# sk4161/EgoScaler

Hardware: AMD Instinct MI355X
Metric: clips/sec/GPU (8-frame 224^2, 16-token text) fwd+bwd (higher is better)
Workload: dtype bf16

## Files before the change

egoscaler_amd/csrc/api.hip:

```cpp
#include "common.h"

thread_local int egomi_launch_err_ = 0;
thread_local int egomi_last_hip_error_ = 0;

extern "C" int egomi_version(void) { return 100; }

extern "C" const char* egomi_last_launch_error(void) { return hipGetErrorString((hipError_t)egomi_last_hip_error_); }

extern "C" const char* egomi_strerror(int code) {
    switch (code) {
        case EGOMI_OK: return "ok";
        case EGOMI_E_BADARG: return "bad argument (null pointer, unknown dtype/enum)";
        case EGOMI_E_SHAPE: return "shape/stride/workspace check failed";
        case EGOMI_E_LAUNCH: return "HIP launch failed";
        case EGOMI_E_UNSUPPORTED: return "size or mode not supported by this kernel";
        default: return "unknown egomi error";
    }
}

thread_local hipEvent_t egomi_time_start_ = nullptr, egomi_time_stop_ = nullptr;

extern "C" int egomi_event_create(void** event) {
    if (!event) return EGOMI_E_BADARG;
    hipEvent_t e;
// ... 5 lines not shown
extern "C" int egomi_event_destroy(void* event) {
    if (!event) return EGOMI_E_BADARG;
    return hipEventDestroy((hipEvent_t)event) == hipSuccess ? EGOMI_OK : EGOMI_E_LAUNCH;
}
extern "C" int egomi_event_elapsed_ms(void* start, void* stop, float* ms) {
    if (!start || !stop || !ms) return EGOMI_E_BADARG;
    hipError_t rc = hipEventSynchronize((hipEvent_t)stop);
    if (rc == hipSuccess) rc = hipEventElapsedTime(ms, (hipEvent_t)start, (hipEvent_t)stop);
    if (rc != hipSuccess) {
        egomi_last_hip_error_ = (int)rc;
        (void)hipGetLastError();
        return EGOMI_E_LAUNCH;
    }
    return EGOMI_OK;
}
thread_local int egomi_route_[5] = {0, 1, 0, 0, 0};

extern "C" int egomi_gemm_last_route(int* out4) {
    if (!out4) return EGOMI_E_BADARG;
    for (int i = 0; i < 4; ++i) out4[i] = egomi_route_[i + 1];
    return egomi_route_[0];
}

extern "C" int egomi_gemm_time_next(void* start, void* stop) {
    if ((start == nullptr) != (stop == nullptr)) return EGOMI_E_BADARG;
    egomi_time_start_ = (hipEvent_t)start; egomi_time_stop_ = (hipEvent_t)stop;
    return EGOMI_OK;
}
```

egoscaler_amd/csrc/common.h:

```cpp
#pragma once
#include <hip/hip_runtime.h>
#include <stdint.h>
#include "../../include/egomi.h"

typedef uint16_t bf16_t;
typedef __attribute__((ext_vector_type(8))) __bf16 bf16x8;
typedef __attribute__((ext_vector_type(4))) __bf16 bf16x4;
typedef __attribute__((ext_vector_type(4))) float f32x4;
typedef __attribute__((ext_vector_type(16))) float f32x16;
typedef __attribute__((ext_vector_type(4))) uint32_t u32x4;
typedef __attribute__((ext_vector_type(2))) uint32_t u32x2;
typedef __attribute__((ext_vector_type(2))) float f32x2;

#define EGOMI_WAVE 64

__device__ __forceinline__ float bf2f(bf16_t u) { return __uint_as_float(((uint32_t)u) << 16); }
__device__ __forceinline__ bf16_t f2bf(float f) {
    __bf16 h = (__bf16)f;
    return *reinterpret_cast<bf16_t*>(&h);
}

__device__ __forceinline__ void swiglu_bwd_elem(float d, float g, float u, float& og, float& ou) {
#pragma clang fp contract(off)
    const float sg = 1.0f / (1.0f + __expf(-g));
// ... 69 lines not shown
    if ((threadIdx.x & 63) == 0) red[w] = v;
    __syncthreads();
    float t = red[0];
    for (int i = 1; i < nw; ++i) t = fmaxf(t, red[i]);
    return t;
}

__device__ __forceinline__ float act_apply(float x, int act) {
    if (act == 1) return 0.5f * x * (1.0f + erff(x * 0.70710678118654752440f));
    if (act == 2) return fmaxf(x, 0.0f);
    return x;
}

extern thread_local int egomi_launch_err_;
extern thread_local int egomi_last_hip_error_;
#define EGOMI_LAUNCH(...)                                              \
    do {                                                               \
        (void)hipGetLastError();                                       \
        hipLaunchKernelGGL(__VA_ARGS__);                               \
        const hipError_t e_ = hipGetLastError();                       \
        if (e_ != hipSuccess) { egomi_launch_err_ = 1; egomi_last_hip_error_ = (int)e_; } \
    } while (0)
extern thread_local int egomi_route_[5];
static inline void egomi_route_set(int form, int splitk, int row0, int slices, int na) {
    egomi_route_[0] = form; egomi_route_[1] = splitk; egomi_route_[2] = row0; egomi_route_[3] = slices; egomi_route_[4] = na;
}
static inline int egomi_launch_status() {
    const int e = egomi_launch_err_;
    egomi_launch_err_ = 0;
    return e ? EGOMI_E_LAUNCH : EGOMI_OK;
}

#define EGOMI_DISPATCH_DTYPE(dtype, ...)                         \
    do {                                                         \
        if ((dtype) == EGOMI_F32) { typedef float T; __VA_ARGS__; }        \
        else if ((dtype) == EGOMI_BF16) { typedef bf16_t T; __VA_ARGS__; } \
        else return EGOMI_E_BADARG;                              \
    } while (0)
```

egoscaler_amd/csrc/gemm.hip:

```cpp
#include "common.h"

#define GT_BM 128
#define GT_BN 128
#define GT_THREADS 256

template <typename T> struct GemmCfg;
template <> struct GemmCfg<bf16_t> { static constexpr int BK = 64, VEC = 8, LDK = 72; };
template <> struct GemmCfg<float> { static constexpr int BK = 16, VEC = 4, LDK = 17; };

struct GemmArgs {
    const void* A; const void* B; void* C; const void* bias; const void* residual;
    int M, N, K;
    long long lda, ldb, ldc, ldr;
    int batch_inner;
    long long sA0, sA1, sB0, sB1, sC0, sC1;
    float alpha; int accumulate; int act;
};


template <typename T, bool TR, int ROWS>
struct Stager {
    static constexpr int BK = GemmCfg<T>::BK, VEC = GemmCfg<T>::VEC, LDK = GemmCfg<T>::LDK;
    static constexpr int NV = ROWS * BK / VEC / GT_THREADS;
    T v[NV][VEC];
// ... 140 lines not shown
    g.alpha = d->alpha; g.accumulate = d->accumulate; g.act = d->act;
    constexpr int VEC = GemmCfg<T>::VEC;
    auto aligned = [&](const void* p, long long ld, long long s0, long long s1) {
        return ((uintptr_t)p % 16 == 0) && (ld % VEC == 0) && (s0 % VEC == 0) && (s1 % VEC == 0);
    };
    const bool aa = aligned(d->A, d->lda, d->sA0, d->sA1), ba = aligned(d->B, d->ldb, d->sB0, d->sB1);
    dim3 grid((d->N + GT_BN - 1) / GT_BN, (d->M + GT_BM - 1) / GT_BM, d->batch > 0 ? d->batch : 1);
    dim3 block(GT_THREADS);
    const bool TA = d->a_layout == 1, TB = d->b_layout == 1;
    if (!TA && !TB) EGOMI_LAUNCH((gemm_generic_kernel<T, TC, false, false>), grid, block, 0, s, g, aa, ba);
    else if (!TA && TB) EGOMI_LAUNCH((gemm_generic_kernel<T, TC, false, true>), grid, block, 0, s, g, aa, ba);
    else if (TA && !TB) EGOMI_LAUNCH((gemm_generic_kernel<T, TC, true, false>), grid, block, 0, s, g, aa, ba);
    else EGOMI_LAUNCH((gemm_generic_kernel<T, TC, true, true>), grid, block, 0, s, g, aa, ba);
    egomi_route_set(1, 1, d->M, 0, 0);
    return egomi_launch_status();
}

int egomi_gemm_fast_try(const egomi_gemm_desc* d, hipStream_t s);
int egomi_gemm_tn_try(const egomi_gemm_desc* d, hipStream_t s);
extern thread_local hipEvent_t egomi_time_start_, egomi_time_stop_;

extern "C" int egomi_gemm(const egomi_gemm_desc* d, egomi_stream_t stream) {
    egomi_route_set(0, 1, d ? d->M : 0, 0, 0);
    if (!d || !d->A || !d->B || !d->C) return EGOMI_E_BADARG;
    if (d->M <= 0 || d->N <= 0 || d->K <= 0) return EGOMI_E_SHAPE;
    if (d->a_layout < 0 || d->a_layout > 1 || d->b_layout < 0 || d->b_layout > 1 || d->act < 0 || d->act > 2) return EGOMI_E_BADARG;
    const long long min_lda = d->a_layout == 0 ? d->K : d->M, min_ldb = d->b_layout == 0 ? d->K : d->N;
    if (d->lda < min_lda || d->ldb < min_ldb || d->ldc < d->N || (d->residual && d->ldr < d->N)) return EGOMI_E_SHAPE;
    if (d->batch > 65535) return EGOMI_E_UNSUPPORTED;
    hipStream_t s = (hipStream_t)stream;
    if (!d->force_generic) {
        const int r = egomi_gemm_fast_try(d, s);
        if (r <= 0) return r;
        const int r2 = egomi_gemm_tn_try(d, s);
        if (r2 <= 0) return r2;
    } else {
        egomi_time_start_ = egomi_time_stop_ = nullptr;
    }
    if (d->epilogue != EGOMI_EPI_NONE) return EGOMI_E_UNSUPPORTED;
    if (d->ab_dtype == EGOMI_F32 && d->c_dtype == EGOMI_F32) return launch_generic<float, float>(d, s);
    if (d->ab_dtype == EGOMI_BF16 && d->c_dtype == EGOMI_BF16) return launch_generic<bf16_t, bf16_t>(d, s);
    if (d->ab_dtype == EGOMI_BF16 && d->c_dtype == EGOMI_F32) return launch_generic<bf16_t, float>(d, s);
    return EGOMI_E_UNSUPPORTED;
}
```

egoscaler_amd/csrc/gemm_fast.hip:

```cpp
#include "common.h"
#include <mutex>
#include <queue>
#include <unordered_map>
#include <vector>

#define FT_BK 64

struct FastArgs {
    const bf16_t* A; const bf16_t* B; void* C; const bf16_t* bias; const void* residual;
    int M, N, K;
    long long lda, ldb, ldc, ldr;
    float alpha; int accumulate; int act;
    int tiles_m, tiles_n;
    int splitk; float* ws;
    int full_tm, full_tiles, tail_s;
    int epi; void* C2; long long ldc2;
    int* tickets;
};

typedef __attribute__((address_space(3))) void lds_void;
typedef __attribute__((address_space(1))) const void gbl_void;

__device__ __forceinline__ void glds16(const bf16_t* g, bf16_t* lds_wave_base) {
    __builtin_amdgcn_global_load_lds((gbl_void*)g, (lds_void*)lds_wave_base, 16, 0, 0);
// ... 388 lines not shown
                for (int i = 0; i < 4; ++i)
                    acc[j][i] = __builtin_amdgcn_mfma_f32_16x16x32_bf16(fb[ks][j], fa[ks][i], acc[j][i], 0, 0, 0);
    }
    asm volatile("s_waitcnt vmcnt(0)" ::: "memory");
    gemm_epilogue<TC, 4>(g, acc, wm, n0 + wn, lane, g.splitk > 1 ? g.ws + (long long)blockIdx.y * g.M * g.N : nullptr, 0);
}

#ifdef GEMM_STAMP
__device__ unsigned long long g_gemm_stamp[16];
extern "C" int egomi_gemm_stamp_read(unsigned long long* out) { return (int)hipMemcpyFromSymbol(out, HIP_SYMBOL(g_gemm_stamp), sizeof(g_gemm_stamp)); }
extern "C" int egomi_gemm_stamp_reset() { unsigned long long z[16] = {0}; return (int)hipMemcpyToSymbol(HIP_SYMBOL(g_gemm_stamp), z, sizeof(z)); }
#define GSTAMP_DECL unsigned long long gs_prev = 0, gs_acc[6] = {0, 0, 0, 0, 0, 0};
#define GSTAMP_NOW(var) { __builtin_amdgcn_sched_barrier(0); asm volatile("s_memtime %0\n\ts_waitcnt lgkmcnt(0)" : "=s"(var) :: "memory"); __builtin_amdgcn_sched_barrier(0); }
#define GSTAMP_START GSTAMP_NOW(gs_prev)
#define GSTAMP(i) { unsigned long long gs_n; GSTAMP_NOW(gs_n) gs_acc[i] += gs_n - gs_prev; gs_prev = gs_n; }
#define GSTAMP_FLUSH if (threadIdx.x == 0) { for (int i = 0; i < 6; ++i) atomicAdd(&g_gemm_stamp[i], gs_acc[i]); atomicAdd(&g_gemm_stamp[8], 1ull); }
#else
#define GSTAMP_DECL
#define GSTAMP_START
#define GSTAMP(i)
#define GSTAMP_FLUSH
#endif
#define P8_HT (128 * 64)
template <typename TC>
__global__ __launch_bounds__(512, 2)
void gemm_nt_bf16_8phase_kernel(FastArgs g) {
    __shared__ __attribute__((aligned(16))) bf16_t smem[2 * 4 * P8_HT];
    const int lane = threadIdx.x & 63;
    const int wave = __builtin_amdgcn_readfirstlane(threadIdx.x >> 6);
    const int wr = wave >> 2, wc = wave & 3;

    GSTAMP_DECL
    GSTAMP_START
    int tm, tn, kz = 0, ksl = 1;
    if ((int)blockIdx.x < g.full_tiles) {
        const int nwg = g.full_tiles;
        int bid = blockIdx.x;
        const int xcd = bid & 7, q = nwg >> 3, r = nwg & 7;
        bid = (xcd < r ? xcd * (q + 1) : r * (q + 1) + (xcd - r) * q) + (bid >> 3);
        const int per_group = 8 * g.tiles_n;
        const int grp = bid / per_group, first_tm = grp * 8;
        const int gsz = (g.full_tm - first_tm) < 8 ? (g.full_tm - first_tm) : 8;
        const int in_g = bid - grp * per_group;
        tm = first_tm + in_g % gsz; tn = in_g / gsz;
    } else {
        const int idx = blockIdx.x - g.full_tiles, rows = g.tiles_m - g.full_tm;
        ksl = g.tail_s;
        kz = idx % ksl;
        const int tile = idx / ksl;
        tm = g.full_tm + tile % rows; tn = tile / rows;
    }
    const int m0 = tm * 256, n0 = tn * 256;

    unsigned offA[2][2], offB[2][2];
#pragma unroll
    for (int h = 0; h < 2; ++h)
#pragma unroll
        for (int i = 0; i < 2; ++i) {
            const int lr = (wave * 2 + i) * 8 + (lane >> 3);
            const int chunk = (lane & 7) ^ ((lr >> 1) & 7);
            int ra = m0 + (lr >> 6) * 128 + h * 64 + (lr & 63); ra = ra < g.M ? ra : g.M - 1;
            int rb = n0 + (lr >> 5) * 64 + h * 32 + (lr & 31);  rb = rb < g.N ? rb : g.N - 1;
            offA[h][i] = (unsigned)(ra * g.lda + chunk * 8);
            offB[h][i] = (unsigned)(rb * g.ldb + chunk * 8);
        }

    f32x4 acc[4][8];
#pragma unroll
    for (int j = 0; j < 4; ++j)
#pragma unroll
        for (int i = 0; i < 8; ++i) acc[j][i] = (f32x4){0.f, 0.f, 0.f, 0.f};

    const int sw = ((lane & 15) >> 1) & 7, c0 = lane >> 4;
    int aBase[2], bBase[2];
#pragma unroll
    for (int ks = 0; ks < 2; ++ks) {
        aBase[ks] = (wr * 64 + (lane & 15)) * 64 + (((c0 + 4 * ks) ^ sw) << 3);
        bBase[ks] = (wc * 32 + (lane & 15)) * 64 + (((c0 + 4 * ks) ^ sw) << 3);
    }

    int nt = g.K / FT_BK, t_begin = 0;
    if (ksl > 1) {
        const int per = (nt + ksl - 1) / ksl;
        t_begin = kz * per;
        nt = t_begin + per < nt ? t_begin + per : nt;
    }
    const int t_last = nt - 1;

    bf16x8 fa[2][4], fb0[2][2], fb1[2][2];

#define P8_RD(off) (*reinterpret_cast<const bf16x8*>(smem + (off)))
#define P8_LDA(b, X) _Pragma("unroll") for (int ks = 0; ks < 2; ++ks) _Pragma("unroll") for (int ii = 0; ii < 4; ++ii) \
        fa[ks][ii] = P8_RD(((b) * 4 + (X)) * P8_HT + aBase[ks] + ii * 16 * 64);
#define P8_LDB(dst, b, X) _Pragma("unroll") for (int ks = 0; ks < 2; ++ks) _Pragma("unroll") for (int jj = 0; jj < 2; ++jj) \
        dst[ks][jj] = P8_RD(((b) * 4 + 2 + (X)) * P8_HT + bBase[ks] + jj * 16 * 64);
#define P8_PF(b, slot, base, off) _Pragma("unroll") for (int i = 0; i < 2; ++i) \
        glds16((base) + (off)[i], smem + ((b) * 4 + (slot)) * P8_HT + (wave * 2 + i) * 8 * 64);
#define P8_MMA(mh, fbv, nh) __builtin_amdgcn_s_setprio(1); \
        _Pragma("unroll") for (int ks = 0; ks < 2; ++ks) _Pragma("unroll") for (int jj = 0; jj < 2; ++jj) _Pragma("unroll") for (int ii = 0; ii < 4; ++ii) \
            acc[(nh) * 2 + jj][(mh) * 4 + ii] = __builtin_amdgcn_mfma_f32_16x16x32_bf16(fbv[ks][jj], fa[ks][ii], acc[(nh) * 2 + jj][(mh) * 4 + ii], 0, 0, 0); \
        __builtin_amdgcn_s_setprio(0);
#define P8_BAR __builtin_amdgcn_sched_barrier(0); __builtin_amdgcn_s_barrier(); __builtin_amdgcn_sched_barrier(0);
#define P8_TILE(b, tt) { \
        const int t1 = (tt) + 1 < t_last ? (tt) + 1 : t_last, t2 = (tt) + 2 < t_last ? (tt) + 2 : t_last; \
        const bf16_t* pA1 = g.A + (long long)t1 * FT_BK; \
        const bf16_t* pA2 = g.A + (long long)t2 * FT_BK; \
        const bf16_t* pB2 = g.B + (long long)t2 * FT_BK; \
         P8_LDB(fb0, b, 0) __builtin_amdgcn_sched_barrier(0); P8_LDA(b, 0) P8_PF((b) ^ 1, 1, pA1, offA[1]) \
        asm volatile("s_waitcnt lgkmcnt(8)" ::: "memory"); P8_BAR P8_MMA(0, fb0, 0) P8_BAR \
         P8_LDB(fb1, b, 1) P8_PF(b, 2, pB2, offB[0]) P8_BAR P8_MMA(0, fb1, 1) P8_BAR \
         P8_LDA(b, 1) P8_PF(b, 0, pA2, offA[0]) P8_BAR P8_MMA(1, fb1, 1) P8_BAR \
         P8_PF(b, 3, pB2, offB[1]) asm volatile("s_waitcnt vmcnt(6)" ::: "memory"); P8_BAR P8_MMA(1, fb0, 0) P8_BAR \
    }

    {
        const int t1 = t_begin + 1 < t_last ? t_begin + 1 : t_last;
        const bf16_t* pA0 = g.A + (long long)t_begin * FT_BK;
        const bf16_t* pB0 = g.B + (long long)t_begin * FT_BK;
        const bf16_t* pA1 = g.A + (long long)t1 * FT_BK;
        const bf16_t* pB1 = g.B + (long long)t1 * FT_BK;
        P8_PF(0, 2, pB0, offB[0]) P8_PF(0, 0, pA0, offA[0]) P8_PF(0, 3, pB0, offB[1]) P8_PF(0, 1, pA0, offA[1])
        P8_PF(1, 2, pB1, offB[0]) P8_PF(1, 0, pA1, offA[0]) P8_PF(1, 3, pB1, offB[1])
        GSTAMP(0)
        asm volatile("s_waitcnt vmcnt(6)" ::: "memory");
        P8_BAR
        GSTAMP(1)
    }
    if (wr == 1) { P8_BAR }
    int t = t_begin;
    for (; t + 1 < nt; t += 2) {
        P8_TILE(0, t)
        P8_TILE(1, t + 1)
    }
    if (t < nt) P8_TILE(0, t)
    if (wr == 0) { P8_BAR }
    GSTAMP(2)
    asm volatile("s_waitcnt vmcnt(0)" ::: "memory");
    __builtin_amdgcn_s_barrier();
    GSTAMP(3)
    const int row0 = g.full_tm * 256;
    const int mb = m0 + wr * 128, nb = n0 + wc * 64;
    if (ksl > 1 && g.tickets) {
        const int tile = (blockIdx.x - g.full_tiles) / ksl;
        char* slab = reinterpret_cast<char*>(g.ws) + (long long)tile * ksl * 262144;
        {
            __amdgpu_buffer_rsrc_t r = __builtin_amdgcn_make_buffer_rsrc(slab + ((long long)kz * 8 + wave) * 32768, 0, 32768, 0x00020000);
#pragma unroll
            for (int j = 0; j < 4; ++j)
#pragma unroll
                for (int i = 0; i < 8; ++i)
                    __builtin_amdgcn_raw_buffer_store_b128(__builtin_bit_cast(u32x4, acc[j][i]), r, ((j * 8 + i) * 64 + lane) * 16, 0, 16);
        }
        int* flag = reinterpret_cast<int*>(smem);
        asm volatile("s_waitcnt vmcnt(0)" ::: "memory");
        __builtin_amdgcn_s_barrier();
        if (threadIdx.x == 0) *flag = __hip_atomic_fetch_add(g.tickets + tile, 1, __ATOMIC_RELAXED, __HIP_MEMORY_SCOPE_AGENT);
        asm volatile("s_waitcnt vmcnt(0) lgkmcnt(0)" ::: "memory");
        __builtin_amdgcn_s_barrier();
        const int tk = *const_cast<volatile int*>(flag);
        if (tk != ksl - 1) return;
        if (threadIdx.x == 0) __hip_atomic_store(g.tickets + tile, 0, __ATOMIC_RELAXED, __HIP_MEMORY_SCOPE_AGENT);
        const bool all = ksl > 2;
        if (all) {
#pragma unroll
            for (int j = 0; j < 4; ++j)
// ... 7 lines not shown
            for (int j = 0; j < 4; ++j)
#pragma unroll
                for (int i = 0; i < 8; ++i)
                    acc[j][i] += __builtin_bit_cast(f32x4, __builtin_amdgcn_raw_buffer_load_b128(r, ((j * 8 + i) * 64 + lane) * 16, 0, 16));
        }
        gemm_epilogue<TC, 8>(g, acc, mb, nb, lane);
        return;
    }
    if (sizeof(TC) == 2 && ksl == 1 && !g.bias && !g.residual && !g.accumulate && g.act == 0 && g.alpha == 1.0f &&
        nb + 64 <= g.N && (g.ldc & 7) == 0 && ((uintptr_t)g.C & 15) == 0) {
        char* wb = reinterpret_cast<char*>(smem) + wave * (64 * 144);
        bf16_t* C = reinterpret_cast<bf16_t*>(g.C);
        if (g.epi == 3) {
            char* ws3 = reinterpret_cast<char*>(smem) + wave * (32 * 272);
            const bf16_t* GU = reinterpret_cast<const bf16_t*>(g.C2);
            const int lr = lane >> 4, ch = lane & 15;
            u32x4 in[8];
#define P8_GU_FETCH(sp_) _Pragma("unroll") for (int it = 0; it < 8; ++it) { \
                    int m_ = mb + (sp_) * 32 + it * 4 + lr; \
                    m_ = m_ < g.M ? m_ : g.M - 1; \
                    in[it] = *reinterpret_cast<const u32x4*>(GU + (long long)m_ * g.ldc2 + 2 * nb + ch * 8); }
            P8_GU_FETCH(0)
#pragma unroll
            for (int sp = 0; sp < 4; ++sp) {
#pragma unroll
                for (int it = 0; it < 8; ++it) *reinterpret_cast<u32x4*>(ws3 + (it * 4 + lr) * 272 + ch * 16) = in[it];
                if (sp < 3) { P8_GU_FETCH(sp + 1) }
#pragma unroll
                for (int i2 = 0; i2 < 2; ++i2)
#pragma unroll
                    for (int j = 0; j < 4; ++j) {
                        const f32x4 v = acc[j][2 * sp + i2];
                        char* pg = ws3 + (i2 * 16 + (lane & 15)) * 272 + ((j >> 1) * 64 + (j & 1) * 16 + lr * 4) * 2;
                        const u32x2 gg = *reinterpret_cast<const u32x2*>(pg), uu = *reinterpret_cast<const u32x2*>(pg + 64);
                        float og[4], ou[4];
#pragma unroll
                        for (int r = 0; r < 4; ++r) {
                            const float gv = __uint_as_float((r & 1) ? (gg[r >> 1] & 0xFFFF0000u) : (gg[r >> 1] << 16));
                            const float uv = __uint_as_float((r & 1) ? (uu[r >> 1] & 0xFFFF0000u) : (uu[r >> 1] << 16));
                            swiglu_bwd_elem(bf2f(f2bf(v[r])), gv, uv, og[r], ou[r]);
                        }
                        u32x2 o;
                        o[0] = (uint32_t)f2bf(og[0]) | ((uint32_t)f2bf(og[1]) << 16);
                        o[1] = (uint32_t)f2bf(og[2]) | ((uint32_t)f2bf(og[3]) << 16);
                        *reinterpret_cast<u32x2*>(pg) = o;
                        o[0] = (uint32_t)f2bf(ou[0]) | ((uint32_t)f2bf(ou[1]) << 16);
                        o[1] = (uint32_t)f2bf(ou[2]) | ((uint32_t)f2bf(ou[3]) << 16);
                        *reinterpret_cast<u32x2*>(pg + 64) = o;
                    }
#pragma unroll
                for (int it = 0; it < 8; ++it) {
                    const int m = mb + sp * 32 + it * 4 + lr;
                    const u32x4 v = *reinterpret_cast<const u32x4*>(ws3 + (it * 4 + lr) * 272 + ch * 16);
                    if (m < g.M) *reinterpret_cast<u32x4*>(C + (long long)m * g.ldc + 2 * nb + ch * 8) = v;
                }
            }
#undef P8_GU_FETCH
            GSTAMP(4)
            GSTAMP(5)
            GSTAMP_FLUSH
            return;
        }
#pragma unroll
        for (int pass = 0; pass < 2; ++pass) {
#pragma unroll
            for (int ii = 0; ii < 4; ++ii)
#pragma unroll
                for (int j = 0; j < 4; ++j) {
                    const f32x4 v = acc[j][4 * pass + ii];
                    u32x2 o;
                    o[0] = (uint32_t)f2bf(v[0]) | ((uint32_t)f2bf(v[1]) << 16);
                    o[1] = (uint32_t)f2bf(v[2]) | ((uint32_t)f2bf(v[3]) << 16);
                    *reinterpret_cast<u32x2*>(wb + (ii * 16 + (lane & 15)) * 144 + (j * 16 + (lane >> 4) * 4) * 2) = o;
                }
#pragma unroll
            for (int it = 0; it < 8; ++it) {
                const int r = it * 8 + (lane >> 3), ch = lane & 7;
                const u32x4 v = *reinterpret_cast<const u32x4*>(wb + r * 144 + ch * 16);
                const int m = mb + pass * 64 + r;
                if (m < g.M) *reinterpret_cast<u32x4*>(C + (long long)m * g.ldc + nb + ch * 8) = v;
            }
            if (g.epi == 1) {
                bf16_t* C2 = reinterpret_cast<bf16_t*>(g.C2);
#pragma unroll
                for (int ii = 0; ii < 4; ++ii)
#pragma unroll
                    for (int j = 0; j < 2; ++j) {
// ... 7 lines not shown
                        }
                        u32x2 o;
                        o[0] = (uint32_t)f2bf(o4[0]) | ((uint32_t)f2bf(o4[1]) << 16);
                        o[1] = (uint32_t)f2bf(o4[2]) | ((uint32_t)f2bf(o4[3]) << 16);
                        *reinterpret_cast<u32x2*>(wb + (ii * 16 + (lane & 15)) * 144 + (j * 16 + (lane >> 4) * 4) * 2) = o;
                    }
#pragma unroll
                for (int it = 0; it < 4; ++it) {
                    const int r = it * 16 + (lane >> 2), ch = lane & 3;
                    const u32x4 v = *reinterpret_cast<const u32x4*>(wb + r * 144 + ch * 16);
                    const int m = mb + pass * 64 + r;
                    if (m < g.M) *reinterpret_cast<u32x4*>(C2 + (long long)m * g.ldc2 + (nb >> 1) + ch * 8) = v;
                }
            }
        }
        GSTAMP(4)
#ifdef GEMM_STAMP
        asm volatile("s_waitcnt vmcnt(0)" ::: "memory");
#endif
        GSTAMP(5)
        GSTAMP_FLUSH
        return;
    }
    gemm_epilogue<TC, 8>(g, acc, mb, nb, lane, ksl > 1 ? g.ws + (long long)kz * (g.M - row0) * g.N : nullptr, row0);
#undef P8_TILE
#undef P8_BAR
#undef P8_MMA
#undef P8_PF
#undef P8_LDB
#undef P8_LDA
#undef P8_RD
}


#define TL_NB 11
#define TL_BM (32 * TL_NB)
#define TL_AB (TL_BM * 128)
#define TL_BUFB (TL_AB + 256 * 128)
__device__ __forceinline__ void tl_dma(const char* gbase, uint32_t voff, uint32_t lds_base) {
    asm volatile("s_mov_b32 m0, %2\n\ts_nop 0\n\tglobal_load_lds_dwordx4 %0, %1" :: "v"(voff), "s"(gbase), "s"(lds_base) : "memory");
}
typedef __attribute__((ext_vector_type(4))) __bf16 tl_bf16x4;
typedef __attribute__((address_space(3))) tl_bf16x4 tl_lds_bf16x4;
template <typename TC, bool TBK>
__global__ __launch_bounds__(512, 2)
void gemm_nt_bf16_tall_kernel(FastArgs g) {
    __shared__ __attribute__((aligned(16))) char smem[2 * TL_BUFB];
    const int lane = threadIdx.x & 63;
    const int wave = __builtin_amdgcn_readfirstlane(threadIdx.x >> 6);
    const int wr = wave >> 2, wc = wave & 3;

// ... 617 lines not shown
        const int ci = ((c >> 5) << 6) + (c & 31);
        float gv[8], uv[8], og[8], ou[8];
        load8<bf16_t>(GU + (long long)m * g.ldc2 + ci, gv);
        load8<bf16_t>(GU + (long long)m * g.ldc2 + ci + 32, uv);
#pragma unroll
        for (int r = 0; r < 8; ++r) swiglu_bwd_elem(bf2f(f2bf(d[r])), gv[r], uv[r], og[r], ou[r]);
        store8<bf16_t>(DGU + (long long)m * g.ldc + ci, og);
        store8<bf16_t>(DGU + (long long)m * g.ldc + ci + 32, ou);
    }
}

static bool fast_applicable(const egomi_gemm_desc* d) {
    if (d->ab_dtype != EGOMI_BF16 || d->a_layout != 0 || d->b_layout != 0) return false;
    if (d->batch > 1) return false;
    if (d->K % FT_BK || d->K < FT_BK) return false;
    if (d->lda % 8 || d->ldb % 8) return false;
    if (((uintptr_t)d->A | (uintptr_t)d->B) & 15) return false;
    const int esz = d->c_dtype == EGOMI_BF16 ? 2 : 4;
    if (((uintptr_t)d->C % (4 * esz)) || (d->residual && ((uintptr_t)d->residual % (4 * esz)))) return false;
    if ((long long)d->M * d->N < 128 * 128) return false;
    return true;
}

static int tile_choice(const egomi_gemm_desc* d) {
    static int forced = -1;
    if (forced < 0) { const char* e = getenv("EGOMI_GEMM_TILE"); forced = e ? atoi(e) : 0; }
    if (forced == 1 || forced == 2 || forced == 8) return forced;
    const long long t256 = (long long)((d->M + 255) / 256) * ((d->N + 255) / 256);
    if (t256 >= 128 && d->K >= 2048 && (long long)d->M * d->lda < (1ll << 31) && (long long)d->N * d->ldb < (1ll << 31)) return 8;
    if (t256 >= 512 && d->K >= 1024 && (long long)d->M * d->lda < (1ll << 31) && (long long)d->N * d->ldb < (1ll << 31)) return 8;
    if (t256 >= 32 && t256 < 128 && d->K >= 8192 && d->M > 512 && d->epilogue == EGOMI_EPI_NONE && d->workspace &&
        d->workspace_bytes >= (long long)((d->M + 255) / 256) * 256 * d->N * 4 * 2 + 4096 &&
        (long long)d->M * d->lda < (1ll << 31) && (long long)d->N * d->ldb < (1ll << 31)) return 8;
    if (d->split_k == 1 && t256 >= 32 && t256 < 128 && d->K >= 2048 && d->M > 512 &&
        (long long)d->M * d->lda < (1ll << 31) && (long long)d->N * d->ldb < (1ll << 31)) return 8;
    return (d->M >= 2048 && d->N >= 8192) ? 2 : 1;
}

extern "C" int egomi_gemm_tn_kernel_id(const egomi_gemm_desc* d);
extern "C" int egomi_gemm_kernel_id(const egomi_gemm_desc* d) {
    if (!d) return EGOMI_E_BADARG;
    if (!d->force_generic && !fast_applicable(d)) return egomi_gemm_tn_kernel_id(d);
    if (d->force_generic || !fast_applicable(d)) return 0;
    return tile_choice(d) == 8 ? 2 : 1;
}

static bool slabs_form_ok(const egomi_gemm_desc* d);
static int skinny_splitk(const egomi_gemm_desc* d, int nwg);
static bool gemv_form(const egomi_gemm_desc* d);
static int gemv_splitk(const egomi_gemm_desc* d);
static bool m256_form(const egomi_gemm_desc* d) {
    static int on = -1;
    if (on < 0) { const char* e = getenv("EGOMI_GEMM_M256"); on = e ? atoi(e) : 1; }
    return on && d->M > 128 && d->M <= 256 && d->N >= 8192 && d->K >= 1024;
}
static int m256_splitk(const egomi_gemm_desc* d) {
    const int nwg = (d->N + 127) / 128, nt = d->K / FT_BK;
// ... 70 lines not shown
    if (g.splitk > 1 && d->epilogue != EGOMI_EPI_SLABS) {
        const long long total = (long long)d->M * ((d->N + 3) / 4);
        const int grid = (int)((total + 255) / 256 < 4096 ? (total + 255) / 256 : 4096);
        if (d->c_dtype == EGOMI_BF16) EGOMI_LAUNCH(splitk_reduce_kernel<bf16_t>, dim3(grid), dim3(256), 0, s, g);
        else EGOMI_LAUNCH(splitk_reduce_kernel<float>, dim3(grid), dim3(256), 0, s, g);
    }
    egomi_route_set(5, g.splitk, d->M, 0, 0);
    return egomi_launch_status();
}

template <int BM, int BN>
static int launch_fast(const egomi_gemm_desc* d, FastArgs& g, hipStream_t s) {
    if (BM == 128 && BN == 128 && gemv_form(d)) return launch_gemv(d, g, s);
    if (BM == 128 && BN == 128 && m256_form(d)) return launch_m256(d, g, s);
    g.tiles_m = (d->M + BM - 1) / BM; g.tiles_n = (d->N + BN - 1) / BN;
    const int nwg = g.tiles_m * g.tiles_n;
    constexpr int threads = (BM / 64) * (BN / 64) * 64;
    g.ws = (float*)d->workspace;
    g.splitk = skinny_splitk(d, nwg);
    if (d->epilogue == EGOMI_EPI_SLABS && g.splitk < 2) return EGOMI_E_UNSUPPORTED;
    static int pf_env = -1;
    if (pf_env < 0) { const char* e = getenv("EGOMI_GEMM_PF"); pf_env = e ? atoi(e) : 1; }
    if (d->c_dtype != EGOMI_BF16 && d->c_dtype != EGOMI_F32) return EGOMI_E_UNSUPPORTED;
    if (BM == 128 && BN == 128 && pf_env) {
        if constexpr (BM == 128 && BN == 128) {
            if (d->c_dtype == EGOMI_BF16) EGOMI_LAUNCH((gemm_nt_bf16_kernel<bf16_t, 128, 128, 2>), dim3(nwg, g.splitk), dim3(threads), 0, s, g);
            else EGOMI_LAUNCH((gemm_nt_bf16_kernel<float, 128, 128, 2>), dim3(nwg, g.splitk), dim3(threads), 0, s, g);
        }
    } else if (d->c_dtype == EGOMI_BF16) EGOMI_LAUNCH((gemm_nt_bf16_kernel<bf16_t, BM, BN, 1>), dim3(nwg, g.splitk), dim3(threads), 0, s, g);
    else EGOMI_LAUNCH((gemm_nt_bf16_kernel<float, BM, BN, 1>), dim3(nwg, g.splitk), dim3(threads), 0, s, g);
    if (g.splitk > 1 && d->epilogue != EGOMI_EPI_SLABS) {
        const long long total = (long long)d->M * ((d->N + 3) / 4);
        const int grid = (int)((total + 255) / 256 < 4096 ? (total + 255) / 256 : 4096);
        if (d->c_dtype == EGOMI_BF16) EGOMI_LAUNCH(splitk_reduce_kernel<bf16_t>, dim3(grid), dim3(256), 0, s, g);
        else EGOMI_LAUNCH(splitk_reduce_kernel<float>, dim3(grid), dim3(256), 0, s, g);
    }
    egomi_route_set(BM == 256 ? 3 : 2, g.splitk, d->M, 0, 0);
    return egomi_launch_status();
}

struct TailPlan { int rows, s; };
static TailPlan plan_tail(int M, int N, int K, long long ws_bytes) {
    static std::mutex mu;
    static std::unordered_map<unsigned long long, TailPlan> cache;
    const unsigned long long key = ((unsigned long long)M << 42) ^ ((unsigned long long)N << 21) ^ (unsigned long long)K ^ (ws_bytes ? 1ull << 63 : 0);
    {
// ... 186 lines not shown
    *row0 = d0->M; *slices = 0;
    egomi_gemm_desc dl = *d0;
    dl.epilogue = EGOMI_EPI_SLABS;
    if (dl.force_generic || !fast_applicable(&dl) || tile_choice(&dl) != 8) return EGOMI_E_UNSUPPORTED;
    if (dl.bias || dl.accumulate || dl.act != 0 || dl.alpha != 1.0f || dl.c_dtype != EGOMI_BF16 || (dl.N & 7)) return EGOMI_E_UNSUPPORTED;
    if (dl.ws_tickets_zeroed && dl.workspace) {
        if (dl.workspace_bytes > 4096) { dl.workspace = (char*)dl.workspace + 4096; dl.workspace_bytes -= 4096; }
        else { dl.workspace = nullptr; dl.workspace_bytes = 0; }
    }
    if (tall_form(&dl)) return EGOMI_OK;
    const TailPlan tp = tail_plan_for(&dl);
    if (tp.rows) { *row0 = ((dl.M + 255) / 256 - tp.rows) * 256; *slices = tp.s; }
    return EGOMI_OK;
}

static int launch_8phase(const egomi_gemm_desc* d, FastArgs& g, hipStream_t s, int* tickets = nullptr, hipEvent_t t0 = nullptr, hipEvent_t t1 = nullptr,
                         bool leave_slabs = false) {
    g.tiles_m = (d->M + 255) / 256; g.tiles_n = (d->N + 255) / 256;
    g.splitk = 1; g.ws = (float*)d->workspace;
    const TailPlan tp = tail_plan_for(d);
    g.full_tm = g.tiles_m - tp.rows; g.tail_s = tp.s; g.full_tiles = g.full_tm * g.tiles_n;
    g.tickets = nullptr;
    if (tp.rows && tickets && tp.rows * g.tiles_n <= 1024 && (long long)tp.rows * g.tiles_n * tp.s * 262144 <= d->workspace_bytes) g.tickets = tickets;
    const int nwg = g.full_tiles + tp.rows * g.tiles_n * tp.s;
    if (d->c_dtype != EGOMI_BF16 && d->c_dtype != EGOMI_F32) return EGOMI_E_UNSUPPORTED;
    if (t0) (void)hipEventRecord(t0, s);
    if (d->c_dtype == EGOMI_BF16) EGOMI_LAUNCH(gemm_nt_bf16_8phase_kernel<bf16_t>, dim3(nwg, 1), dim3(512), 0, s, g);
    else EGOMI_LAUNCH(gemm_nt_bf16_8phase_kernel<float>, dim3(nwg, 1), dim3(512), 0, s, g);
    if (t1) (void)hipEventRecord(t1, s);
    egomi_route_set(6, 1, tp.rows ? g.full_tm * 256 : d->M, tp.rows ? tp.s : 0, 0);
    if (tp.rows && g.epi == 1 && g.tickets) g.tickets = nullptr;
    if (leave_slabs) return egomi_launch_status();
    if (tp.rows && g.epi == 3) {
        FastArgs r = g;
        const long long row0 = (long long)g.full_tm * 256;
        r.M = d->M - (int)row0; r.splitk = tp.s;
        r.C = (char*)g.C + row0 * g.ldc * 2;
        r.C2 = (char*)g.C2 + row0 * g.ldc2 * 2;
        const long long total = (long long)r.M * (d->N / 8);
        const int grid = (int)((total + 255) / 256 < 4096 ? (total + 255) / 256 : 4096);
        EGOMI_LAUNCH(splitk_reduce_swiglu_bwd_kernel, dim3(grid), dim3(256), 0, s, r);
        return egomi_launch_status();
    }
    if (tp.rows && !g.tickets) {
        FastArgs r = g;
        const long long row0 = (long long)g.full_tm * 256;
        const int esz = d->c_dtype == EGOMI_BF16 ? 2 : 4;
        r.M = d->M - (int)row0; r.splitk = tp.s;
        r.C = (char*)g.C + row0 * g.ldc * esz;
        if (g.residual) r.residual = (const char*)g.residual + row0 * g.ldr * esz;
        const long long total = (long long)r.M * ((d->N + 3) / 4);
// ... 134 lines not shown
```

egoscaler_amd/ops.py:

```python
import ctypes
import math

import torch

from . import _abi, _lib
from ._lib import c_p, c_i, c_d, c_f, c_sz, c_i64, call, query

F32, BF16 = _abi.EGOMI_F32, _abi.EGOMI_BF16


def dt(t: torch.dtype) -> int:
    if t == torch.float32:
        return F32
    if t == torch.bfloat16:
        return BF16
    raise TypeError(f"unsupported dtype {t}")


def P(t):
    if t is None:
        return c_p(None)
    if not t.is_cuda:
        raise _lib.EgomiError("egoscaler_amd ops need CUDA/HIP tensors (no CPU fallback)")
    return c_p(t.data_ptr())
# ... 397 lines not shown
def mm_kernel_id(a, b, out, a_layout=0, b_layout=0, accumulate=False):
    M, K = (a.shape if a_layout == 0 else (a.shape[1], a.shape[0]))
    N = b.shape[0] if b_layout == 0 else b.shape[1]
    d = GemmDesc()
    d.A, d.B, d.C = a.data_ptr(), b.data_ptr(), out.data_ptr()
    d.M, d.N, d.K, d.lda, d.ldb, d.ldc = M, N, K, _ld(a), _ld(b), _ld(out)
    d.a_layout, d.b_layout, d.ab_dtype, d.c_dtype, d.batch = a_layout, b_layout, dt(a.dtype), dt(out.dtype), 1
    d.alpha, d.accumulate = 1.0, int(accumulate)
    return query("egomi_gemm_kernel_id", ctypes.byref(d))


GEMM_FORMS = {0: "none", 1: "generic", 2: "128x128", 3: "256x128", 4: "gemv_m16", 5: "m256", 6: "8phase", 7: "persistent", 8: "tall",
              9: "split", 10: "kmajor", 11: "kmajor_tall", 12: "kmajor_split"}


def gemm_last_route():
    out = (c_i * 4)()
    form = query("egomi_gemm_last_route", out)
    if form < 0:
        _lib.check(form, "egomi_gemm_last_route")
    return (GEMM_FORMS[form],) + tuple(out)


def swiglu_bwd(dact, gate, up, dgate, dup):
    rows, cols = gate.shape
    call("egomi_swiglu_bwd", dact, gate, up, dgate, dup, rows, cols, _ld(gate), _ld(dact), _ld(dgate), dt(gate.dtype), S())


def gelu(x, out=None):
    out = torch.empty_like(x) if out is None else out
    call("egomi_gelu_fwd", x, out, x.numel(), dt(x.dtype), S())
    return out


def gelu_bwd(dy, x, out=None):
    out = torch.empty_like(x) if out is None else out
    call("egomi_gelu_bwd", dy, x, out, x.numel(), dt(x.dtype), S())
    return out


def softmax(scores, Z, heads, Sq, Sk, out, causal=False, q_offset=0, key_mask=None):
    call("egomi_softmax_fwd", scores, Sk, key_mask, Z, heads, Sq, Sk, int(causal), q_offset, out, Sk, dt(out.dtype), S())
    return out


def softmax_bwd(Pm, dP, dS, rows, Sk):
# ... 233 lines not shown
```

include/egomi.h:

```cpp
#ifndef EGOMI_H
#define EGOMI_H
#include <stddef.h>
#include <stdint.h>

#ifdef __cplusplus
extern "C" {
#endif

#define EGOMI_OK 0
#define EGOMI_E_BADARG (-1)
#define EGOMI_E_SHAPE (-2)
#define EGOMI_E_LAUNCH (-3)
#define EGOMI_E_UNSUPPORTED (-4)

#define EGOMI_F32 0
#define EGOMI_BF16 1

typedef void* egomi_stream_t;

int egomi_version(void);
const char* egomi_strerror(int code);
const char* egomi_last_launch_error(void);

size_t egomi_unproject_workspace_bytes(int B, int T, int H, int W);
// ... 17 lines not shown
typedef struct egomi_gemm_desc {
    const void* A; const void* B; void* C; const void* bias; const void* residual;
    int M, N, K;
    int64_t lda, ldb, ldc, ldr;
    int a_layout, b_layout;
    int ab_dtype, c_dtype;
    int batch, batch_inner;
    int64_t sA0, sA1, sB0, sB1, sC0, sC1;
    float alpha;
    int accumulate;
    int act;
    int force_generic;
    void* workspace; int64_t workspace_bytes; int split_k;
    int ws_tickets_zeroed;
    int epilogue; void* C2; int64_t ldc2;
} egomi_gemm_desc;
#define EGOMI_EPI_NONE 0
#define EGOMI_EPI_SWIGLU 1
#define EGOMI_EPI_SLABS 2
#define EGOMI_EPI_SWIGLU_BWD 3
int egomi_gemm(const egomi_gemm_desc* desc, egomi_stream_t stream);
int egomi_gemm_kernel_id(const egomi_gemm_desc* desc);
int egomi_gemm_set_tall(int mode);
int egomi_gemm_slab_count(const egomi_gemm_desc* desc);
int egomi_gemm_tail_plan(const egomi_gemm_desc* desc, int* row0, int* slices);
int egomi_gemm_tn_tail_plan(const egomi_gemm_desc* desc, int* row0, int* slices);
int egomi_gemm_last_route(int* out4);
#define EGOMI_ROUTE_FORMS 13
int egomi_event_create(void** event);
int egomi_event_destroy(void* event);
int egomi_event_elapsed_ms(void* start, void* stop, float* ms);
int egomi_gemm_time_next(void* start, void* stop);

typedef struct egomi_attn_desc {
    const void* q; const void* k; const void* v; void* o; float* lse;
    const void* dout; float* delta; void* dq; void* dk; void* dv;
    const uint8_t* key_mask;
    int B, H, S, head_dim;
    int64_t ld_qkv, ld_o, ld_dqkv;
    float scale;
    int causal;
    int dtype;
    const float* rope_cos; const float* rope_sin;
    int q_rows;
} egomi_attn_desc;
int egomi_attn_fwd(const egomi_attn_desc* desc, egomi_stream_t stream);
// ... 196 lines not shown
```

Before: 66.47.

## Add 128-row variant of 8-phase GEMM kernel to fill CUs on small grids

```diff
diff --git a/egoscaler_amd/csrc/api.hip b/egoscaler_amd/csrc/api.hip
--- a/egoscaler_amd/csrc/api.hip
+++ b/egoscaler_amd/csrc/api.hip
@@ -51,6 +51,9 @@
     return egomi_route_[0];
 }
 
+thread_local int egomi_tile_rows_ = 0;
+extern "C" int egomi_gemm_last_tile_rows() { return egomi_tile_rows_; }
+
 extern "C" int egomi_gemm_time_next(void* start, void* stop) {
     if ((start == nullptr) != (stop == nullptr)) return EGOMI_E_BADARG;
     egomi_time_start_ = (hipEvent_t)start; egomi_time_stop_ = (hipEvent_t)stop;
diff --git a/egoscaler_amd/csrc/common.h b/egoscaler_amd/csrc/common.h
--- a/egoscaler_amd/csrc/common.h
+++ b/egoscaler_amd/csrc/common.h
@@ -115,6 +115,7 @@
         if (e_ != hipSuccess) { egomi_launch_err_ = 1; egomi_last_hip_error_ = (int)e_; } \
     } while (0)
 extern thread_local int egomi_route_[5];
+extern thread_local int egomi_tile_rows_;
 static inline void egomi_route_set(int form, int splitk, int row0, int slices, int na) {
     egomi_route_[0] = form; egomi_route_[1] = splitk; egomi_route_[2] = row0; egomi_route_[3] = slices; egomi_route_[4] = na;
 }
diff --git a/egoscaler_amd/csrc/gemm.hip b/egoscaler_amd/csrc/gemm.hip
--- a/egoscaler_amd/csrc/gemm.hip
+++ b/egoscaler_amd/csrc/gemm.hip
@@ -186,6 +186,7 @@
 
 extern "C" int egomi_gemm(const egomi_gemm_desc* d, egomi_stream_t stream) {
     egomi_route_set(0, 1, d ? d->M : 0, 0, 0);
+    egomi_tile_rows_ = 0;
     if (!d || !d->A || !d->B || !d->C) return EGOMI_E_BADARG;
     if (d->M <= 0 || d->N <= 0 || d->K <= 0) return EGOMI_E_SHAPE;
     if (d->a_layout < 0 || d->a_layout > 1 || d->b_layout < 0 || d->b_layout > 1 || d->act < 0 || d->act > 2) return EGOMI_E_BADARG;
diff --git a/egoscaler_amd/csrc/gemm_fast.hip b/egoscaler_amd/csrc/gemm_fast.hip
--- a/egoscaler_amd/csrc/gemm_fast.hip
+++ b/egoscaler_amd/csrc/gemm_fast.hip
@@ -434,10 +434,14 @@
 #define GSTAMP_FLUSH
 #endif
 #define P8_HT (128 * 64)
-template <typename TC>
+template <typename TC, int MI>
 __global__ __launch_bounds__(512, 2)
 void gemm_nt_bf16_8phase_kernel(FastArgs g) {
-    __shared__ __attribute__((aligned(16))) bf16_t smem[2 * 4 * P8_HT];
+    constexpr int BM = 64 * MI;
+    constexpr int AH = 32 * MI * 64;
+    constexpr int BUF = 2 * AH + 2 * P8_HT;
+    constexpr int APC = MI / 2;
+    __shared__ __attribute__((aligned(16))) bf16_t smem[2 * BUF];
     const int lane = threadIdx.x & 63;
     const int wave = __builtin_amdgcn_readfirstlane(threadIdx.x >> 6);
     const int wr = wave >> 2, wc = wave & 3;
@@ -462,32 +466,33 @@
         const int tile = idx / ksl;
         tm = g.full_tm + tile % rows; tn = tile / rows;
     }
-    const int m0 = tm * 256, n0 = tn * 256;
-
-    unsigned offA[2][2], offB[2][2];
+    const int m0 = tm * BM, n0 = tn * 256;
+
+    unsigned offA[2][APC], offB[2][2];
 #pragma unroll
     for (int h = 0; h < 2; ++h)
 #pragma unroll
         for (int i = 0; i < 2; ++i) {
             const int lr = (wave * 2 + i) * 8 + (lane >> 3);
             const int chunk = (lane & 7) ^ ((lr >> 1) & 7);
-            int ra = m0 + (lr >> 6) * 128 + h * 64 + (lr & 63); ra = ra < g.M ? ra : g.M - 1;
+            const int la = MI == 4 ? lr : wave * 8 + (lane >> 3);
+            int ra = m0 + (la >> (MI == 4 ? 6 : 5)) * (32 * MI) + h * (16 * MI) + (la & (16 * MI - 1)); ra = ra < g.M ? ra : g.M - 1;
             int rb = n0 + (lr >> 5) * 64 + h * 32 + (lr & 31);  rb = rb < g.N ? rb : g.N - 1;
-            offA[h][i] = (unsigned)(ra * g.lda + chunk * 8);
+            if (i < APC) offA[h][i] = (unsigned)(ra * g.lda + ((lane & 7) ^ ((la >> 1) & 7)) * 8);
             offB[h][i] = (unsigned)(rb * g.ldb + chunk * 8);
         }
 
-    f32x4 acc[4][8];
+    f32x4 acc[4][2 * MI];
 #pragma unroll
     for (int j = 0; j < 4; ++j)
 #pragma unroll
-        for (int i = 0; i < 8; ++i) acc[j][i] = (f32x4){0.f, 0.f, 0.f, 0.f};
+        for (int i = 0; i < 2 * MI; ++i) acc[j][i] = (f32x4){0.f, 0.f, 0.f, 0.f};
 
     const int sw = ((lane & 15) >> 1) & 7, c0 = lane >> 4;
     int aBase[2], bBase[2];
 #pragma unroll
     for (int ks = 0; ks < 2; ++ks) {
-        aBase[ks] = (wr * 64 + (lane & 15)) * 64 + (((c0 + 4 * ks) ^ sw) << 3);
+        aBase[ks] = (wr * (16 * MI) + (lane & 15)) * 64 + (((c0 + 4 * ks) ^ sw) << 3);
         bBase[ks] = (wc * 32 + (lane & 15)) * 64 + (((c0 + 4 * ks) ^ sw) << 3);
     }
 
@@ -499,18 +504,22 @@
     }
     const int t_last = nt - 1;
 
-    bf16x8 fa[2][4], fb0[2][2], fb1[2][2];
+    bf16x8 fa[2][MI], fb0[2][2], fb1[2][2];
 
 #define P8_RD(off) (*reinterpret_cast<const bf16x8*>(smem + (off)))
-#define P8_LDA(b, X) _Pragma("unroll") for (int ks = 0; ks < 2; ++ks) _Pragma("unroll") for (int ii = 0; ii < 4; ++ii) \
-        fa[ks][ii] = P8_RD(((b) * 4 + (X)) * P8_HT + aBase[ks] + ii * 16 * 64);
+#define P8_LDA(b, X) _Pragma("unroll") for (int ks = 0; ks < 2; ++ks) _Pragma("unroll") for (int ii = 0; ii < MI; ++ii) \
+        fa[ks][ii] = P8_RD((b) * BUF + (X) * AH + aBase[ks] + ii * 16 * 64);
 #define P8_LDB(dst, b, X) _Pragma("unroll") for (int ks = 0; ks < 2; ++ks) _Pragma("unroll") for (int jj = 0; jj < 2; ++jj) \
-        dst[ks][jj] = P8_RD(((b) * 4 + 2 + (X)) * P8_HT + bBase[ks] + jj * 16 * 64);
-#define P8_PF(b, slot, base, off) _Pragma("unroll") for (int i = 0; i < 2; ++i) \
-        glds16((base) + (off)[i], smem + ((b) * 4 + (slot)) * P8_HT + (wave * 2 + i) * 8 * 64);
+        dst[ks][jj] = P8_RD((b) * BUF + 2 * AH + (X) * P8_HT + bBase[ks] + jj * 16 * 64);
+#define P8_PFA(b, h, base) _Pragma("unroll") for (int i = 0; i < APC; ++i) \
+        glds16((base) + offA[h][i], smem + (b) * BUF + (h) * AH + (wave * APC + i) * 8 * 64);
+#define P8_PFB(b, h, base) _Pragma("unroll") for (int i = 0; i < 2; ++i) \
+        glds16((base) + offB[h][i], smem + (b) * BUF + 2 * AH + (h) * P8_HT + (wave * 2 + i) * 8 * 64);
+#define P8_WAIT_VM asm volatile("s_waitcnt vmcnt(%0)" :: "n"(4 + APC) : "memory");
+#define P8_WAIT_LGKM asm volatile("s_waitcnt lgkmcnt(%0)" :: "n"(2 * MI) : "memory");
 #define P8_MMA(mh, fbv, nh) __builtin_amdgcn_s_setprio(1); \
-        _Pragma("unroll") for (int ks = 0; ks < 2; ++ks) _Pragma("unroll") for (int jj = 0; jj < 2; ++jj) _Pragma("unroll") for (int ii = 0; ii < 4; ++ii) \
-            acc[(nh) * 2 + jj][(mh) * 4 + ii] = __builtin_amdgcn_mfma_f32_16x16x32_bf16(fbv[ks][jj], fa[ks][ii], acc[(nh) * 2 + jj][(mh) * 4 + ii], 0, 0, 0); \
+        _Pragma("unroll") for (int ks = 0; ks < 2; ++ks) _Pragma("unroll") for (int jj = 0; jj < 2; ++jj) _Pragma("unroll") for (int ii = 0; ii < MI; ++ii) \
+            acc[(nh) * 2 + jj][(mh) * MI + ii] = __builtin_amdgcn_mfma_f32_16x16x32_bf16(fbv[ks][jj], fa[ks][ii], acc[(nh) * 2 + jj][(mh) * MI + ii], 0, 0, 0); \
         __builtin_amdgcn_s_setprio(0);
 #define P8_BAR __builtin_amdgcn_sched_barrier(0); __builtin_amdgcn_s_barrier(); __builtin_amdgcn_sched_barrier(0);
 #define P8_TILE(b, tt) { \
@@ -518,11 +527,11 @@
         const bf16_t* pA1 = g.A + (long long)t1 * FT_BK; \
         const bf16_t* pA2 = g.A + (long long)t2 * FT_BK; \
         const bf16_t* pB2 = g.B + (long long)t2 * FT_BK; \
-         P8_LDB(fb0, b, 0) __builtin_amdgcn_sched_barrier(0); P8_LDA(b, 0) P8_PF((b) ^ 1, 1, pA1, offA[1]) \
-        asm volatile("s_waitcnt lgkmcnt(8)" ::: "memory"); P8_BAR P8_MMA(0, fb0, 0) P8_BAR \
-         P8_LDB(fb1, b, 1) P8_PF(b, 2, pB2, offB[0]) P8_BAR P8_MMA(0, fb1, 1) P8_BAR \
-         P8_LDA(b, 1) P8_PF(b, 0, pA2, offA[0]) P8_BAR P8_MMA(1, fb1, 1) P8_BAR \
-         P8_PF(b, 3, pB2, offB[1]) asm volatile("s_waitcnt vmcnt(6)" ::: "memory"); P8_BAR P8_MMA(1, fb0, 0) P8_BAR \
+         P8_LDB(fb0, b, 0) __builtin_amdgcn_sched_barrier(0); P8_LDA(b, 0) P8_PFA((b) ^ 1, 1, pA1) \
+        P8_WAIT_LGKM P8_BAR P8_MMA(0, fb0, 0) P8_BAR \
+         P8_LDB(fb1, b, 1) P8_PFB(b, 0, pB2) P8_BAR P8_MMA(0, fb1, 1) P8_BAR \
+         P8_LDA(b, 1) P8_PFA(b, 0, pA2) P8_BAR P8_MMA(1, fb1, 1) P8_BAR \
+         P8_PFB(b, 1, pB2) P8_WAIT_VM P8_BAR P8_MMA(1, fb0, 0) P8_BAR \
     }
 
     {
@@ -531,10 +540,10 @@
         const bf16_t* pB0 = g.B + (long long)t_begin * FT_BK;
         const bf16_t* pA1 = g.A + (long long)t1 * FT_BK;
         const bf16_t* pB1 = g.B + (long long)t1 * FT_BK;
-        P8_PF(0, 2, pB0, offB[0]) P8_PF(0, 0, pA0, offA[0]) P8_PF(0, 3, pB0, offB[1]) P8_PF(0, 1, pA0, offA[1])
-        P8_PF(1, 2, pB1, offB[0]) P8_PF(1, 0, pA1, offA[0]) P8_PF(1, 3, pB1, offB[1])
+        P8_PFB(0, 0, pB0) P8_PFA(0, 0, pA0) P8_PFB(0, 1, pB0) P8_PFA(0, 1, pA0)
+        P8_PFB(1, 0, pB1) P8_PFA(1, 0, pA1) P8_PFB(1, 1, pB1)
         GSTAMP(0)
-        asm volatile("s_waitcnt vmcnt(6)" ::: "memory");
+        P8_WAIT_VM
         P8_BAR
         GSTAMP(1)
     }
@@ -550,9 +559,9 @@
     asm volatile("s_waitcnt vmcnt(0)" ::: "memory");
     __builtin_amdgcn_s_barrier();
     GSTAMP(3)
-    const int row0 = g.full_tm * 256;
-    const int mb = m0 + wr * 128, nb = n0 + wc * 64;
-    if (ksl > 1 && g.tickets) {
+    const int row0 = g.full_tm * BM;
+    const int mb = m0 + wr * (32 * MI), nb = n0 + wc * 64;
+    if constexpr (MI == 4) if (ksl > 1 && g.tickets) {
         const int tile = (blockIdx.x - g.full_tiles) / ksl;
         char* slab = reinterpret_cast<char*>(g.ws) + (long long)tile * ksl * 262144;
         {
@@ -606,10 +615,10 @@
                     in[it] = *reinterpret_cast<const u32x4*>(GU + (long long)m_ * g.ldc2 + 2 * nb + ch * 8); }
             P8_GU_FETCH(0)
 #pragma unroll
-            for (int sp = 0; sp < 4; ++sp) {
+            for (int sp = 0; sp < MI; ++sp) {
 #pragma unroll
                 for (int it = 0; it < 8; ++it) *reinterpret_cast<u32x4*>(ws3 + (it * 4 + lr) * 272 + ch * 16) = in[it];
-                if (sp < 3) { P8_GU_FETCH(sp + 1) }
+                if (sp < MI - 1) { P8_GU_FETCH(sp + 1) }
 #pragma unroll
                 for (int i2 = 0; i2 < 2; ++i2)
 #pragma unroll
@@ -646,7 +655,7 @@
             return;
         }
 #pragma unroll
-        for (int pass = 0; pass < 2; ++pass) {
+        for (int pass = 0; pass < MI / 2; ++pass) {
 #pragma unroll
             for (int ii = 0; ii < 4; ++ii)
 #pragma unroll
@@ -700,11 +709,14 @@
         GSTAMP_FLUSH
         return;
     }
-    gemm_epilogue<TC, 8>(g, acc, mb, nb, lane, ksl > 1 ? g.ws + (long long)kz * (g.M - row0) * g.N : nullptr, row0);
+    gemm_epilogue<TC, 2 * MI>(g, acc, mb, nb, lane, ksl > 1 ? g.ws + (long long)kz * (g.M - row0) * g.N : nullptr, row0);
 #undef P8_TILE
 #undef P8_BAR
 #undef P8_MMA
-#undef P8_PF
+#undef P8_WAIT_LGKM
+#undef P8_WAIT_VM
+#undef P8_PFB
+#undef P8_PFA
 #undef P8_LDB
 #undef P8_LDA
 #undef P8_RD
@@ -1368,6 +1380,14 @@
     return true;
 }
 
+static int g_narrow_mode = -1;
+extern "C" int egomi_gemm_set_narrow(int mode) { g_narrow_mode = mode < 0 ? -1 : (mode > 2 ? 2 : mode); return EGOMI_OK; }
+static int narrow_mode() {
+    if (g_narrow_mode < 0) { const char* e = getenv("EGOMI_GEMM_NARROW"); g_narrow_mode = e ? atoi(e) : 1; if (g_narrow_mode < 0 || g_narrow_mode > 2) g_narrow_mode = 1; }
+    return g_narrow_mode;
+}
+static int p8_cus();
+
 static int tile_choice(const egomi_gemm_desc* d) {
     static int forced = -1;
     if (forced < 0) { const char* e = getenv("EGOMI_GEMM_TILE"); forced = e ? atoi(e) : 0; }
@@ -1379,6 +1399,8 @@
         d->workspace_bytes >= (long long)((d->M + 255) / 256) * 256 * d->N * 4 * 2 + 4096 &&
         (long long)d->M * d->lda < (1ll << 31) && (long long)d->N * d->ldb < (1ll << 31)) return 8;
     if (d->split_k == 1 && t256 >= 32 && t256 < 128 && d->K >= 2048 && d->M > 512 &&
+        (long long)d->M * d->lda < (1ll << 31) && (long long)d->N * d->ldb < (1ll << 31)) return 8;
+    if (narrow_mode() == 2 && d->split_k == 1 && d->K >= 2048 && d->epilogue == EGOMI_EPI_NONE &&
         (long long)d->M * d->lda < (1ll << 31) && (long long)d->N * d->ldb < (1ll << 31)) return 8;
     return (d->M >= 2048 && d->N >= 8192) ? 2 : 1;
 }
@@ -1495,6 +1517,7 @@
     static int pf_env = -1;
     if (pf_env < 0) { const char* e = getenv("EGOMI_GEMM_PF"); pf_env = e ? atoi(e) : 1; }
     if (d->c_dtype != EGOMI_BF16 && d->c_dtype != EGOMI_F32) return EGOMI_E_UNSUPPORTED;
+    egomi_tile_rows_ = BM;
     if (BM == 128 && BN == 128 && pf_env) {
         if constexpr (BM == 128 && BN == 128) {
             if (d->c_dtype == EGOMI_BF16) EGOMI_LAUNCH((gemm_nt_bf16_kernel<bf16_t, 128, 128, 2>), dim3(nwg, g.splitk), dim3(threads), 0, s, g);
@@ -1727,11 +1750,19 @@
     g.full_tm = g.tiles_m - tp.rows; g.tail_s = tp.s; g.full_tiles = g.full_tm * g.tiles_n;
     g.tickets = nullptr;
     if (tp.rows && tickets && tp.rows * g.tiles_n <= 1024 && (long long)tp.rows * g.tiles_n * tp.s * 262144 <= d->workspace_bytes) g.tickets = tickets;
+    const int nm = narrow_mode(), tm128 = (d->M + 127) / 128;
+    const bool narrow = !tp.rows && (nm == 2 || (nm == 1 && g.tiles_m * g.tiles_n < p8_cus() && tm128 > g.tiles_m && tm128 * g.tiles_n <= p8_cus()));
+    if (narrow) { g.tiles_m = g.full_tm = tm128; g.full_tiles = tm128 * g.tiles_n; }
+    egomi_tile_rows_ = narrow ? 128 : 256;
     const int nwg = g.full_tiles + tp.rows * g.tiles_n * tp.s;
     if (d->c_dtype != EGOMI_BF16 && d->c_dtype != EGOMI_F32) return EGOMI_E_UNSUPPORTED;
     if (t0) (void)hipEventRecord(t0, s);
-    if (d->c_dtype == EGOMI_BF16) EGOMI_LAUNCH(gemm_nt_bf16_8phase_kernel<bf16_t>, dim3(nwg, 1), dim3(512), 0, s, g);
-    else EGOMI_LAUNCH(gemm_nt_bf16_8phase_kernel<float>, dim3(nwg, 1), dim3(512), 0, s, g);
+    if (narrow) {
+        if (d->c_dtype == EGOMI_BF16) EGOMI_LAUNCH((gemm_nt_bf16_8phase_kernel<bf16_t, 2>), dim3(nwg, 1), dim3(512), 0, s, g);
+        else EGOMI_LAUNCH((gemm_nt_bf16_8phase_kernel<float, 2>), dim3(nwg, 1), dim3(512), 0, s, g);
+    }
+    else if (d->c_dtype == EGOMI_BF16) EGOMI_LAUNCH((gemm_nt_bf16_8phase_kernel<bf16_t, 4>), dim3(nwg, 1), dim3(512), 0, s, g);
+    else EGOMI_LAUNCH((gemm_nt_bf16_8phase_kernel<float, 4>), dim3(nwg, 1), dim3(512), 0, s, g);
     if (t1) (void)hipEventRecord(t1, s);
     egomi_route_set(6, 1, tp.rows ? g.full_tm * 256 : d->M, tp.rows ? tp.s : 0, 0);
     if (tp.rows && g.epi == 1 && g.tickets) g.tickets = nullptr;
diff --git a/egoscaler_amd/ops.py b/egoscaler_amd/ops.py
--- a/egoscaler_amd/ops.py
+++ b/egoscaler_amd/ops.py
@@ -443,6 +443,14 @@
     return (GEMM_FORMS[form],) + tuple(out)
 
 
+def gemm_set_narrow(mode):
+    call("egomi_gemm_set_narrow", mode)
+
+
+def gemm_last_tile_rows():
+    return query("egomi_gemm_last_tile_rows")
+
+
 def swiglu_bwd(dact, gate, up, dgate, dup):
     rows, cols = gate.shape
     call("egomi_swiglu_bwd", dact, gate, up, dgate, dup, rows, cols, _ld(gate), _ld(dact), _ld(dgate), dt(gate.dtype), S())
diff --git a/include/egomi.h b/include/egomi.h
--- a/include/egomi.h
+++ b/include/egomi.h
@@ -63,6 +63,8 @@
 int egomi_gemm(const egomi_gemm_desc* desc, egomi_stream_t stream);
 int egomi_gemm_kernel_id(const egomi_gemm_desc* desc);
 int egomi_gemm_set_tall(int mode);
+int egomi_gemm_set_narrow(int mode);
+int egomi_gemm_last_tile_rows(void);
 int egomi_gemm_slab_count(const egomi_gemm_desc* desc);
 int egomi_gemm_tail_plan(const egomi_gemm_desc* desc, int* row0, int* slices);
 int egomi_gemm_tn_tail_plan(const egomi_gemm_desc* desc, int* row0, int* slices);
```

New measurement: 66.30. No clear change (-0.3%).
